# tp7/Sushi

Measured on NVIDIA H100. Metric: subtitle_events_per_s, higher is better.
Workload: dtype f32

## Files before the change

### sushi_b200/csrc/sb_fused2.cu

```cuda
#include "sb_internal.h"
#include <cmath>
#include <cstdlib>
#include <vector>

#include "sb_fused_common.cuh"
#include "sb_fft_smem.cuh"

using namespace sb;
using namespace sbf;

#ifndef SB_V2_SPECIAL_PREFETCH
#define SB_V2_SPECIAL_PREFETCH 1
#endif

namespace {

constexpr int QB = 16384;
constexpr int QT = 512;
constexpr int QNW = QT / 32;
constexpr int Q4 = QB / 4;
constexpr int QBLK = 256;
constexpr int QROW = kQuadRowF2 / 2;
__host__ __device__ constexpr int qa(int i) { return i < Q4 ? (i >> 8) * (2 * QBLK) + (i & (QBLK - 1)) : 2 * Q4; }
__host__ __device__ constexpr int qm(int i) { return i < Q4 ? qa(i) + QBLK : 2 * Q4 + 1; }
// ... 379 lines not shown
        int rq = 0, rs = 0;
        double dq = 0.0, ds = 0.0;
#pragma unroll
        for (int i = 0; i < 8; ++i) {
            const float wq = f_w0q + (is_u8 ? (float)rq : (float)dq);
            const float sit = fmaf(cc[i], f_scale, fmaf(f_b, is_u8 ? (float)rs : (float)ds, f_k0));
            const float num = fmaxf((wq + f_tsq) - 2.0f * sit, 0.0f);
            const float pr = wq * f_tsq;
            const float v = fminf(num * rsqrt_fast(pr), 1.0f);
            if (interior) { vf[c][i] = v; tmin = fminf(tmin, v); }
            else if (j0 + i >= jlo && j0 + i < jhi) { vf[c][i] = v; tmin = fminf(tmin, v); }
            else vf[c][i] = kSent;
            if (is_u8) {
                const int lo = (int)((lo8 >> (8 * i)) & 0xffu), hi = (int)((hi8 >> (8 * i)) & 0xffu);
                rq += hi * hi - lo * lo; rs += hi - lo;
            } else if (j0 + i + n < img_n) {
                const double lo = (double)img32[j0 + i], hi = (double)img32[j0 + i + n];
                dq += hi * hi - lo * lo; ds += hi - lo;
            }
        }
    }
    const float my_min = tmin;
#pragma unroll
    for (int o = 16; o > 0; o >>= 1) tmin = fminf(tmin, __shfl_xor_sync(0xffffffffu, tmin, o));
    if (lane == 0) s_min[warp] = tmin;
    if (is_u8) fence_proxy_async();
    csync<ID>();
    after_read();
    float bmin = s_min[0];
#pragma unroll
    for (int w = 1; w < NW; ++w) bmin = fminf(bmin, s_min[w]);
    const float thr = curve_out ? 1.5f : bmin + kScreenMargin;

    unsigned long long cand = 0;
    if (my_min <= thr) {
#pragma unroll
        for (int c = 0; c < ROUNDS; ++c)
#pragma unroll
            for (int i = 0; i < 8; ++i) cand |= (vf[c][i] <= thr) ? (1ull << (c * 8 + i)) : 0ull;
    }
    unsigned long long best = ~0ull;
    while (cand) {
        const int bit = __ffsll((long long)cand) - 1;
        cand &= cand - 1;
        const int m = (bit >> 3) * LAGS_PER_ROUND + tid * 8 + (bit & 7);
        const int64_t j = j_blk + m;
        const int jj = m >> 2;
        const int ca = (jj & 15) * kDA + ((jj >> 4) & 15) * kDB + 2 * (jj >> 8);
        const C2 E = buf.ld(ca), O = buf.ld(ca + 1);
        const float2 w = make_float2(kC32[jj >> 8], kS32[jj >> 8]);
        const bool second = (m & 2) != 0;
        const float er = second ? E.r.y : E.r.x, ei = second ? E.i.y : E.i.x, orr = second ? O.r.y : O.r.x, oi = second ? O.i.y : O.i.x;
        const float xr = fmaf(orr, w.x, fmaf(oi, -w.y, er)), xi = fmaf(orr, w.y, fmaf(oi, w.x, ei));
        const double cc = (double)((m & 1) ? xi : xr) * scale;
        const double2 p_hi = ipfx[j + n], p_lo = ipfx[j];
        const float v = sqdiff_exact(cc, p_hi.x - p_lo.x, p_hi.y - p_lo.y, a, b, tsum, tsq, n_ab);
        if (curve_out) curve_out[d.curveOff + (j - jlo)] = v;
        const unsigned long long key = ((unsigned long long)__float_as_uint(v) << 32) | (unsigned int)(j - jlo);
        best = key < best ? key : best;
    }
#pragma unroll
    for (int o = 16; o > 0; o >>= 1) {
        const unsigned long long other = __shfl_xor_sync(0xffffffffu, best, o);
        best = other < best ? other : best;
    }
    if (lane == 0) s_best[warp] = best;
    csync<ID>();
    if (tid == 0) {
        for (int w = 1; w < NW; ++w) best = s_best[w] < best ? s_best[w] : best;
        if (best != ~0ull) atomicMin(keys + it.q, best);
    }
}

template <int ID, typename AfterRead>
__device__ __forceinline__ void finish_item_v3(const Item& it, int tid, const Smem& sm, unsigned long long* s_bar, unsigned bar_parity,
                                               float* s_min, int2* s_w0, int64_t img_n,
                                               unsigned long long* __restrict__ keys, float* __restrict__ curve_out,
                                               AfterRead after_read, RunSink sink) {
    constexpr int NW = QNW, LB = QB, RUNS = 4;
    constexpr float kSent = 3.0e38f;
    const Buf& buf = sm.buf;
    const int lane = tid & 31, warp = tid >> 5;
    const QueryDesc& d = it.d;
    const int64_t j_blk = it.j_blk, n = d.tlen, jlo = d.lag0, jhi = d.lag0 + d.nlags;
    const double2* s_qc = reinterpret_cast<const double2*>(sm.end + kQueryConstOff());
    const double tsum = s_qc[0].x, tsq = s_qc[0].y, a = s_qc[1].x, b = s_qc[1].y;
    const double n_ab = (double)n * a * b;
    const double scale = 1.0 / (double)(2 * QB);
    const double k_const = a * tsum - n_ab;
    const float f_tsq = (float)tsq, f_b = (float)b;
    const float m2s = -2.0f * (float)scale, m2b = -2.0f * f_b;
    const bool interior = j_blk >= jlo && j_blk + LB <= jhi;
    const int64_t jt = j_blk + 32 * tid;
    constexpr float kRunQ = 7.0f * 255.0f * 255.0f;
    const float f_bm = fmaxf(f_b, 255.0f - f_b);
    const float f_delta = 1.02f * 7.0f * f_bm * f_bm + 1024.0f;
    const float rt = sqrtf(f_tsq), m_rt = kScreenMargin * rt, sat = (1.0f - kScreenMargin) * rt;
    const int ech = 8 * (tid & 1) * kDA + ((tid >> 1) & 15) * kDB + 2 * warp;
    const float wc = kC32[warp], ws = kS32[warp];

    mbar_wait(s_bar, bar_parity);
    unsigned lw[8], hw[8];
    {
        const uint4 l0 = *reinterpret_cast<const uint4*>(sm.lo + 32 * tid), l1 = *reinterpret_cast<const uint4*>(sm.lo + 32 * tid + 16);
        lw[0] = l0.x; lw[1] = l0.y; lw[2] = l0.z; lw[3] = l0.w; lw[4] = l1.x; lw[5] = l1.y; lw[6] = l1.z; lw[7] = l1.w;
        const int hi_off = (int)((j_blk + n) & 15);
        const uint4 h0 = *reinterpret_cast<const uint4*>(sm.hi + 32 * tid), h1 = *reinterpret_cast<const uint4*>(sm.hi + 32 * tid + 16),
                    h2 = *reinterpret_cast<const uint4*>(sm.hi + 32 * tid + 32);
        unsigned w[12] = {h0.x, h0.y, h0.z, h0.w, h1.x, h1.y, h1.z, h1.w, h2.x, h2.y, h2.z, h2.w};
        unsigned v[10], u[9];
#pragma unroll
        for (int k = 0; k < 10; ++k) v[k] = (hi_off & 8) ? w[k + 2] : w[k];
#pragma unroll
        for (int k = 0; k < 9; ++k) u[k] = (hi_off & 4) ? v[k + 1] : v[k];
        const unsigned sh = (unsigned)(hi_off & 3) * 8u;
#pragma unroll
        for (int k = 0; k < 8; ++k) hw[k] = __funnelshift_r(u[k], u[k + 1], sh);
    }
    int tq[RUNS], ts[RUNS];
#pragma unroll
    for (int r = 0; r < RUNS; ++r) {
        tq[r] = (int)__dp4a(hw[2 * r], hw[2 * r], __dp4a(hw[2 * r + 1], hw[2 * r + 1], 0u)) - (int)__dp4a(lw[2 * r], lw[2 * r], __dp4a(lw[2 * r + 1], lw[2 * r + 1], 0u));
        ts[r] = (int)__dp4a(hw[2 * r], 0x01010101u, __dp4a(hw[2 * r + 1], 0x01010101u, 0u)) - (int)__dp4a(lw[2 * r], 0x01010101u, __dp4a(lw[2 * r + 1], 0x01010101u, 0u));
    }
    const int Tq = (tq[0] + tq[1]) + (tq[2] + tq[3]), Ts = (ts[0] + ts[1]) + (ts[2] + ts[3]);
    int iq = Tq, is = Ts;
#pragma unroll
    for (int o = 1; o < 32; o <<= 1) {
        const int uq = __shfl_up_sync(0xffffffffu, iq, o), us = __shfl_up_sync(0xffffffffu, is, o);
        if (lane >= o) { iq += uq; is += us; }
    }
    const double2 b_lo = sm.base[warp * 2], b_hi = sm.base[warp * 2 + 1];
    const double Wq = b_hi.y - b_lo.y, Ws = b_hi.x - b_lo.x;
    const double Cw = Wq + tsq - 2.0 * (b * Ws + k_const);
    const int bi2 = 2 * (int)b;
    float run_lb[RUNS];
    float tmin = kSent;
    int oq = iq - Tq, os = is - Ts;
#pragma unroll
    for (int r = 0; r < RUNS; ++r) {
        s_w0[r * QT + tid] = make_int2(os, oq);
        const float f_w0q = (float)(Wq + 0.25 + (double)oq);
        const float f_A = (float)(Cw + (double)(oq - bi2 * os));
        float cc[8];
#pragma unroll
        for (int e = 0; e < 2; ++e) {
            const C2 E = buf.ld(ech + kDA * (2 * r + e)), O = buf.ld(ech + kDA * (2 * r + e) + 1);
            const float2 xr = fma2(O.r, bc(wc), fma2(O.i, bc(-ws), E.r));
            const float2 xi = fma2(O.r, bc(ws), fma2(O.i, bc(wc), E.i));
            cc[4 * e + 0] = xr.x; cc[4 * e + 1] = xi.x; cc[4 * e + 2] = xr.y; cc[4 * e + 3] = xi.y;
        }
        const float cmax = fmaxf(fmaxf(fmaxf(cc[0], cc[1]), fmaxf(cc[2], cc[3])), fmaxf(fmaxf(cc[4], cc[5]), fmaxf(cc[6], cc[7])));
        const int64_t j0 = jt + 8 * r;
        const bool some = interior || (j0 < jhi && j0 + 8 > jlo);
        const bool inside = interior || (j0 >= jlo && j0 + 8 <= jhi);
        const float lbn = fmaf(cmax, m2s, f_A - f_delta), ubn = lbn + 2.0f * f_delta;
        const float lbv = lbn * rsqrt_fast(f_w0q + kRunQ) * 0.999999f;
        run_lb[r] = !some ? kSent : (lbn >= 0.f ? lbv : -kSent);
        const float ubv = ubn * rsqrt_fast(f_w0q - kRunQ) * 1.000001f;
        if (inside && f_w0q > 4.0f * kRunQ && ubn >= 0.f) tmin = fminf(tmin, ubv);
        oq += tq[r]; os += ts[r];
    }
#pragma unroll
    for (int o = 16; o > 0; o >>= 1) tmin = fminf(tmin, __shfl_xor_sync(0xffffffffu, tmin, o));
    if (lane == 0) s_min[warp] = tmin;
    fence_proxy_async();
    csync<ID>();
    static_assert(NW == 16, "block minimum over 16 warps");
    float bmin = s_min[lane & (NW - 1)];
#pragma unroll
    for (int o = NW / 2; o > 0; o >>= 1) bmin = fminf(bmin, __shfl_xor_sync(0xffffffffu, bmin, o));
    const float thr = bmin + m_rt;
    const bool all = curve_out != nullptr || !(bmin < sat);
    unsigned left = 0;
#pragma unroll
    for (int r = 0; r < RUNS; ++r) left |= (run_lb[r] <= thr || (all && run_lb[r] < kSent)) ? (1u << r) : 0u;
    if (left && sink.recs != nullptr && !all) {
#pragma unroll 1
        for (int r = 0; r < RUNS; ++r) {
            if (!((left >> r) & 1u)) continue;
            const int slot = atomicAdd(sink.s_cnt, 1);
            if (slot >= kRunSlots) break;
            float cc[8];
            const int k3 = warp;
#pragma unroll
            for (int e = 0; e < 2; ++e) {
                const C2 E = buf.ld(ech + kDA * (2 * r + e)), O = buf.ld(ech + kDA * (2 * r + e) + 1);
                const float2 w = make_float2(kC32[k3], kS32[k3]);
                const float2 xr = fma2(O.r, bc(w.x), fma2(O.i, bc(-w.y), E.r));
                const float2 xi = fma2(O.r, bc(w.y), fma2(O.i, bc(w.x), E.i));
                cc[4 * e + 0] = xr.x; cc[4 * e + 1] = xi.x; cc[4 * e + 2] = xr.y; cc[4 * e + 3] = xi.y;
            }
            float4* r4 = reinterpret_cast<float4*>(sink.recs + slot);
            const int64_t j0 = jt + 8 * r;
            *reinterpret_cast<int4*>(r4) = make_int4(it.q, 1, (int)(unsigned)(j0 & 0xffffffffll), (int)(j0 >> 32));
            r4[1] = make_float4(cc[0], cc[1], cc[2], cc[3]);
            r4[2] = make_float4(cc[4], cc[5], cc[6], cc[7]);
            left &= ~(1u << r);
        }
    }
    unsigned long long best = ~0ull;
    if (__any_sync(0xffffffffu, left != 0u)) {
        unsigned cand = 0;
#pragma unroll 1
        for (int r = 0; r < RUNS; ++r) {
            const bool sel = (left >> r) & 1u;
            if (!__any_sync(0xffffffffu, sel)) continue;
            const int64_t j0 = jt + 8 * r;
            float cc[8];
#pragma unroll
            for (int e = 0; e < 2; ++e) {
                const C2 E = buf.ld(ech + kDA * (2 * r + e)), O = buf.ld(ech + kDA * (2 * r + e) + 1);
                const float2 xr = fma2(O.r, bc(wc), fma2(O.i, bc(-ws), E.r));
                const float2 xi = fma2(O.r, bc(ws), fma2(O.i, bc(wc), E.i));
                cc[4 * e + 0] = xr.x; cc[4 * e + 1] = xi.x; cc[4 * e + 2] = xr.y; cc[4 * e + 3] = xi.y;
            }
            const unsigned long long lo8 = *reinterpret_cast<const unsigned long long*>(sm.lo + 32 * tid + 8 * r);
            const int hb = (int)((j_blk + n) & 15) + 32 * tid + 8 * r;
            const unsigned long long h0 = *reinterpret_cast<const unsigned long long*>(sm.hi + (hb & ~7));
            const unsigned long long h1 = *reinterpret_cast<const unsigned long long*>(sm.hi + (hb & ~7) + 8);
            const unsigned shb = (unsigned)(hb & 7) * 8u;
            const unsigned long long hi8 = shb ? ((h0 >> shb) | (h1 << (64u - shb))) : h0;
            const int2 off = s_w0[r * QT + tid];
            const float f_w0q = (float)(Wq + 0.25 + (double)off.y);
            const float f_A = (float)(Cw + (double)(off.y - bi2 * off.x));
            float v8[8];
            float vmin = kSent;
            int rq = 0, rs = 0;
#pragma unroll
            for (int i = 0; i < 8; ++i) {
                const float frq = (float)rq;
                const float num = fmaf(cc[i], m2s, fmaf(m2b, (float)rs, f_A + frq));
                const float v = num * rsqrt_fast(f_w0q + frq);
                const bool valid = sel && j0 + i >= jlo && j0 + i < jhi;
                v8[i] = valid ? v : kSent;
                vmin = fminf(vmin, v8[i]);
                const int lo = (int)((lo8 >> (8 * i)) & 0xffu), hi = (int)((hi8 >> (8 * i)) & 0xffu);
                const int dd = hi - lo;
                rq += (hi + lo) * dd; rs += dd;
            }
#pragma unroll
            for (int o = 16; o > 0; o >>= 1) vmin = fminf(vmin, __shfl_xor_sync(0xffffffffu, vmin, o));
            const float thrw = fminf(thr, vmin + m_rt);
#pragma unroll
            for (int i = 0; i < 8; ++i) cand |= (v8[i] < kSent && (v8[i] <= thrw || all)) ? (1u << (r * 8 + i)) : 0u;
        }
        while (cand) {
            const int bit = __ffs((int)cand) - 1;
            cand &= cand - 1;
            const int r = bit >> 3, i = bit & 7;
            const int m = 32 * tid + bit;
            const int64_t j = j_blk + m;
            const int jj = m >> 2;
            const int ca = (jj & 15) * kDA + ((jj >> 4) & 15) * kDB + 2 * (jj >> 8);
            const C2 E = buf.ld(ca), O = buf.ld(ca + 1);
            const float2 w = make_float2(kC32[jj >> 8], kS32[jj >> 8]);
            const bool second = (m & 2) != 0;
            const float er = second ? E.r.y : E.r.x, ei = second ? E.i.y : E.i.x, orr = second ? O.r.y : O.r.x, oi = second ? O.i.y : O.i.x;
            const float xr = fmaf(orr, w.x, fmaf(oi, -w.y, er)), xi = fmaf(orr, w.y, fmaf(oi, w.x, ei));
            const double cc = (double)((m & 1) ? xi : xr) * scale;
            const unsigned long long lo8 = *reinterpret_cast<const unsigned long long*>(sm.lo + 32 * tid + 8 * r);
            const int hb = (int)((j_blk + n) & 15) + 32 * tid + 8 * r;
            const unsigned long long h0 = *reinterpret_cast<const unsigned long long*>(sm.hi + (hb & ~7));
            const unsigned long long h1 = *reinterpret_cast<const unsigned long long*>(sm.hi + (hb & ~7) + 8);
            const unsigned shb = (unsigned)(hb & 7) * 8u;
            const unsigned long long hi8 = shb ? ((h0 >> shb) | (h1 << (64u - shb))) : h0;
            const unsigned long long keep = i ? (~0ull >> (8 * (8 - i))) : 0ull;
            const unsigned la = (unsigned)(lo8 & keep), lb = (unsigned)((lo8 & keep) >> 32), ha = (unsigned)(hi8 & keep), hb2 = (unsigned)((hi8 & keep) >> 32);
            const int rq = (int)__dp4a(ha, ha, __dp4a(hb2, hb2, 0u)) - (int)__dp4a(la, la, __dp4a(lb, lb, 0u));
            const int rs = (int)__dp4a(ha, 0x01010101u, __dp4a(hb2, 0x01010101u, 0u)) - (int)__dp4a(la, 0x01010101u, __dp4a(lb, 0x01010101u, 0u));
            const int2 off = s_w0[r * QT + tid];
            const double wsum = (Ws + (double)off.x) + (double)rs, wsq = (Wq + (double)off.y) + (double)rq;
            const float v = sqdiff_exact(cc, wsum, wsq, a, b, tsum, tsq, n_ab);
            if (curve_out) curve_out[d.curveOff + (j - jlo)] = v;
            const unsigned long long key = ((unsigned long long)__float_as_uint(v) << 32) | (unsigned int)(j - jlo);
            best = key < best ? key : best;
        }
        if (best != ~0ull) atomicMin(keys + it.q, best);
    }
    fence_proxy_async();
    csync<ID>();
    after_read();
}

template <typename S> struct QueryStreams { const float4* Xhat; int64_t nblk; const S* img; int64_t img_n; const double2* ipfx; const double2* tpfx; };
template <typename S>
__device__ __forceinline__ QueryStreams<S> select_streams(const StreamEntry* streams, const int2* slots, int q) {
    const int2 sl = slots[q];
    const StreamEntry si = streams[sl.x];
    return {reinterpret_cast<const float4*>(si.specq), si.nblk, static_cast<const S*>(si.raw), si.n, si.pfx, streams[sl.y].pfx};
}
#define SB_SELECT_STREAMS(q) do { const QueryStreams<S> qs__ = select_streams<S>(streams, slots, (q)); \
    Xhat = qs__.Xhat; nblk = qs__.nblk; img = qs__.img; img_n = qs__.img_n; ipfx = qs__.ipfx; tpfx = qs__.tpfx; } while (0)

template <typename S, int EPI, bool MULTI = false>
__global__ void __launch_bounds__(QT, 1)
k_match_packed(const float4* __restrict__ That, int64_t part_first,
               const float4* __restrict__ Xhat, int64_t nblk,
               const S* __restrict__ img, int64_t img_n,
               const double2* __restrict__ ipfx, const double2* __restrict__ tpfx,
               const QueryDesc* __restrict__ desc, const int* __restrict__ item_query, int64_t item_first,
               PackedTables tab, unsigned long long* __restrict__ keys, float* __restrict__ curve_out,
               RunRecord* __restrict__ recs, int* __restrict__ rec_count,
               const StreamEntry* __restrict__ streams = nullptr, const int2* __restrict__ slots = nullptr) {
    constexpr int T = QT, NW = QNW;
    constexpr bool is_u8 = sizeof(S) == 1;
    extern __shared__ __align__(16) unsigned char smem_raw[];
    const Smem sm(smem_raw);
    unsigned long long* s_bar = reinterpret_cast<unsigned long long*>(sm.end);
    unsigned long long* s_best = s_bar + 1;
    float* s_min = reinterpret_cast<float*>(s_best + NW);
    int* s_cnt = reinterpret_cast<int*>(sm.end + kRunCountOff());
    const RunSink sink = {EPI == 3 && recs ? recs + (size_t)blockIdx.x * kRunSlots : nullptr, s_cnt};
    float4* s_sp = reinterpret_cast<float4*>(sm.end + kSmallBytes);
    int2* s_w0 = EPI >= 2 && is_u8 ? reinterpret_cast<int2*>(sm.end + kSmallBytes + kSpecialBytes) : nullptr;
    const Buf& buf = sm.buf;

    const int tid = threadIdx.x, lane = tid & 31, warp = tid >> 5;
    const Item it(desc, item_query, item_first, blockIdx.x);
    const QueryDesc& d = it.d;
    if constexpr (MULTI) SB_SELECT_STREAMS(it.q);

    if (is_u8) {
        if (tid == 0) mbar_init(s_bar, 1);
        stage_inputs<EPI == 3>(it, tid, reinterpret_cast<const uint8_t*>(img), img_n, ipfx, sm, s_bar);
    }
    if (EPI == 3 && tid == 96) *s_cnt = 0;
    if (EPI >= 2 && tid == 64) query_constants<S>(reinterpret_cast<double2*>(sm.end + kQueryConstOff()), d, img_n, ipfx, tpfx);

    {
        int P = d.P;
        if (it.k + P > nblk) P = (int)(nblk - it.k);
        typedef Rows R;
        const float4* tp = That + (d.partBase - part_first) * (int64_t)R::STRIDE;
        const float4* xp = Xhat + it.k * (int64_t)R::STRIDE;
        const float2 wbase = __ldg(tab.wb + tid);
        const int tm = (T - tid) & (T - 1);
        const int col = phys(tid), mcol = phys(tm);
        const bool sp_pref = EPI >= 2 && SB_V2_SPECIAL_PREFETCH && special_fits(d.P, 1);
        if (sp_pref && warp == NW - 1) special_prefetch(s_sp, tp, xp, d.P, 1, it.k, nblk, lane);
        constexpr int U = 4;
#pragma unroll 1
        for (int half = 0; half < 2; ++half) {
            const int i0 = R::unit(tid, half * U);
            QuadAcc acc[U];
#pragma unroll
            for (int u = 0; u < U; ++u) acc[u].zero();
#pragma unroll 1
            for (int p = 0; p < P; ++p) {
                const float4* t = tp + (int64_t)p * R::STRIDE;
                const float4* x = xp + (int64_t)p * R::STRIDE;
                float4 ta[U], tmm[U], xa[U], xm[U];
#pragma unroll
                for (int u = 0; u < U; ++u) {
                    R::load(t, i0 + u * R::USTEP, ta[u], tmm[u]);
                    R::load(x, i0 + u * R::USTEP, xa[u], xm[u]);
                }
#pragma unroll
                for (int u = 0; u < U; ++u) acc[u].mac(ta[u], tmm[u], xa[u], xm[u]);
            }
#pragma unroll
            for (int u = 0; u < U; ++u) {
                const int uu = half * U + u;
                const float c = wbase.x * kC64[uu] - wbase.y * kS64[uu];
                const float s = wbase.x * kS64[uu] + wbase.y * kC64[uu];
                C2 lo, hi;
                pack_quad(acc[u].aR, acc[u].aI, acc[u].mR, acc[u].mI, c, s, lo, hi);
                buf.st(col + kUU * uu, lo);
                if (tid != 0) buf.st(mcol + kUU * (15 - uu), hi);
                else if (uu != 0) buf.st(mcol + kUU * (16 - uu), hi);
            }
        }
        if (warp == NW - 1) {
            if (sp_pref) {
                cp_async_commit_wait_all();
                __syncwarp();
                const C2 lo = special_from_smem(s_sp, d.P, 0, lane);
                if (lane == 0) buf.st(phys(Q4), lo);
            } else {
                const C2 lo = special_quad(tp, xp, P, lane);
                if (lane == 0) buf.st(phys(Q4), lo);
            }
        }
    }
    csync<0>();

    fft_passes_dif<0>(buf, tid, tab, is_u8);
    if constexpr (EPI == 3) finish_item_v3<0>(it, tid, sm, s_bar, 0u, s_min, s_w0, img_n, keys, curve_out, [] {}, sink);
    else finish_item<S, 0>(it, tid, sm, s_bar, 0u, s_best, s_min, img, img_n, ipfx, tpfx, keys, curve_out, [] {});
    if (EPI == 3 && rec_count && tid == 0) rec_count[blockIdx.x] = *s_cnt < kRunSlots ? *s_cnt : kRunSlots;
}

constexpr int kParkF4 = 16 * QT;

__device__ __forceinline__ void unpark(const float4* pk, const Buf& buf, int col, int mcol, int tid) {
#pragma unroll
    for (int uu = 0; uu < 8; ++uu) {
        const C2 lo = from4(park_ld(pk + (2 * uu) * QT)), hi = from4(park_ld(pk + (2 * uu + 1) * QT));
        buf.st(col + kUU * uu, lo);
        if (tid != 0) buf.st(mcol + kUU * (15 - uu), hi);
        else if (uu != 0) buf.st(mcol + kUU * (16 - uu), hi);
    }
}

template <typename S, int EPI, bool MULTI = false>
__global__ void __launch_bounds__(QT, 1)
k_match_pair(const float4* __restrict__ That, int64_t part_first,
             const float4* __restrict__ Xhat, int64_t nblk,
             const S* __restrict__ img, int64_t img_n,
             const double2* __restrict__ ipfx, const double2* __restrict__ tpfx,
             const QueryDesc* __restrict__ desc, const int* __restrict__ pair_query, int64_t pair_first, int64_t n_pairs,
             float4* __restrict__ park, int* __restrict__ park_busy, int park_slots,
             PackedTables tab, unsigned long long* __restrict__ keys, float* __restrict__ curve_out,
             RunRecord* __restrict__ recs, int* __restrict__ rec_count,
             const StreamEntry* __restrict__ streams = nullptr, const int2* __restrict__ slots = nullptr) {
    constexpr int T = QT, NW = QNW;
    constexpr bool is_u8 = sizeof(S) == 1;
    extern __shared__ __align__(16) unsigned char smem_raw[];
    const Smem sm(smem_raw);
    unsigned long long* s_bar = reinterpret_cast<unsigned long long*>(sm.end);
    unsigned long long* s_best = s_bar + 1;
    float* s_min = reinterpret_cast<float*>(s_best + NW);
    int* s_slot = reinterpret_cast<int*>(s_min + NW);
    int* s_cnt = reinterpret_cast<int*>(sm.end + kRunCountOff());
    int* s_next_q = reinterpret_cast<int*>(sm.end + kNextOff());
    QueryDesc* s_next_d = reinterpret_cast<QueryDesc*>(sm.end + kNextOff() + 16);
    float4* s_sp = reinterpret_cast<float4*>(sm.end + kSmallBytes);
    int2* s_w0 = EPI >= 2 && is_u8 ? reinterpret_cast<int2*>(sm.end + kSmallBytes + kSpecialBytes) : nullptr;
    const Buf& buf = sm.buf;

    const int tid = threadIdx.x, lane = tid & 31, warp = tid >> 5;
    if (tid == 64) *s_slot = park_acquire(park_busy, park_slots, (int)(blockIdx.x % (unsigned)park_slots));
    if (is_u8 && tid == 0) mbar_init(s_bar, 1);
    if (EPI == 3 && tid == 32) *s_cnt = 0;
    csync<0>();
    float4* const pk = park + (size_t)*s_slot * kParkF4 + tid;
    const int tm = (T - tid) & (T - 1);
    const int col = phys(tid), mcol = phys(tm);
    const float2 wbase = __ldg(tab.wb + tid);
    unsigned phase = 0;

    constexpr bool kPersistent = EPI == 3, kPrefetch = kPersistent;
    int64_t pi = blockIdx.x;
    do {
    const bool first = !kPrefetch || pi == (int64_t)blockIdx.x;
    const int q = first ? __ldg(pair_query + pi) : *s_next_q;
    const QueryDesc d = first ? desc[q] : *s_next_d;
    if constexpr (MULTI) SB_SELECT_STREAMS(q);
    const int64_t pi_next = pi + gridDim.x;
    int q_next = 0;
    if (kPrefetch && tid == 32 && pi_next < n_pairs) q_next = __ldg(pair_query + pi_next);
    const int lp = (int)(pair_first + pi - d.groupBase);
    const bool has2 = 2 * lp + 1 < d.nk;
    const Item it0(d, q, d.k0 + 2 * lp), it1(d, q, d.k0 + 2 * lp + 1);
    const RunSink sink = {EPI == 3 && recs ? recs + (size_t)pi * kRunSlots : nullptr, s_cnt};

    if (is_u8) stage_inputs<EPI == 3>(it0, tid, reinterpret_cast<const uint8_t*>(img), img_n, ipfx, sm, s_bar);
    if (EPI >= 2 && tid == 64) query_constants<S>(reinterpret_cast<double2*>(sm.end + kQueryConstOff()), d, img_n, ipfx, tpfx);
    C2 sp1 = {make_float2(0.f, 0.f), make_float2(0.f, 0.f)};
    {
        typedef Rows R;
        const int64_t k = it0.k;
        const float4* tp = That + (d.partBase - part_first) * (int64_t)R::STRIDE;
        const float4* xp = Xhat + k * (int64_t)R::STRIDE;
        const bool sp_pref = EPI >= 2 && SB_V2_SPECIAL_PREFETCH && special_fits(d.P, 2);
        if (sp_pref && warp == NW - 1) special_prefetch(s_sp, tp, xp, d.P, 2, k, nblk, lane);
        constexpr int U = 2;
#pragma unroll 1
        for (int grp = 0; grp < 8 / U; ++grp) {
            const int i0 = R::unit(tid, grp * U);
            QuadAcc a0[U], a1[U];
            float4 xa[U], xm[U];
#pragma unroll
            for (int u = 0; u < U; ++u) {
                a0[u].zero(); a1[u].zero();
                R::load(xp, i0 + u * R::USTEP, xa[u], xm[u]);
            }
#pragma unroll 2
            for (int p = 0; p < d.P; ++p) {
                const float4* t = tp + (int64_t)p * R::STRIDE;
                const float4* x = xp + (int64_t)(p + 1) * R::STRIDE;
                const bool next_row = k + p + 1 < nblk;
                float4 ta[U], tmm[U], xna[U], xnm[U];
#pragma unroll
                for (int u = 0; u < U; ++u) {
                    R::load(t, i0 + u * R::USTEP, ta[u], tmm[u]);
                    R::loadp(x, i0 + u * R::USTEP, next_row, xna[u], xnm[u]);
                }
#pragma unroll
                for (int u = 0; u < U; ++u) {
                    a0[u].mac(ta[u], tmm[u], xa[u], xm[u]);
                    a1[u].mac(ta[u], tmm[u], xna[u], xnm[u]);
                    xa[u] = xna[u]; xm[u] = xnm[u];
                }
            }
#pragma unroll
            for (int u = 0; u < U; ++u) {
                const int uu = grp * U + u;
                const float c = wbase.x * kC64[uu] - wbase.y * kS64[uu];
                const float s = wbase.x * kS64[uu] + wbase.y * kC64[uu];
                C2 lo, hi;
                pack_quad(a0[u].aR, a0[u].aI, a0[u].mR, a0[u].mI, c, s, lo, hi);
                buf.st(col + kUU * uu, lo);
                if (tid != 0) buf.st(mcol + kUU * (15 - uu), hi);
                else if (uu != 0) buf.st(mcol + kUU * (16 - uu), hi);
                pack_quad(a1[u].aR, a1[u].aI, a1[u].mR, a1[u].mI, c, s, lo, hi);
                park_st(pk + (2 * uu) * QT, make_float4(lo.r.x, lo.r.y, lo.i.x, lo.i.y));
                park_st(pk + (2 * uu + 1) * QT, make_float4(hi.r.x, hi.r.y, hi.i.x, hi.i.y));
            }
        }
        if (warp == NW - 1) {
            if (sp_pref) {
                cp_async_commit_wait_all();
                __syncwarp();
                const C2 lo = special_from_smem(s_sp, d.P, 0, lane);
                if (lane == 0) buf.st(phys(Q4), lo);
                if (has2) sp1 = special_from_smem(s_sp, d.P, 1, lane);
            } else {
                int P0 = d.P; if (k + P0 > nblk) P0 = (int)(nblk - k);
                const C2 lo = special_quad(tp, xp, P0, lane);
                if (lane == 0) buf.st(phys(Q4), lo);
                if (has2) {
                    int P1 = d.P; if (k + 1 + P1 > nblk) P1 = (int)(nblk - k - 1);
                    sp1 = special_quad(tp, xp + R::STRIDE, P1, lane);
                }
            }
        }
    }
    csync<0>();
    if (kPrefetch && tid == 32 && pi_next < n_pairs) {
        *s_next_q = q_next;
        const float4* src = reinterpret_cast<const float4*>(desc + q_next);
        static_assert(sizeof(QueryDesc) == 80, "five 16-byte copies");
#pragma unroll
        for (int k = 0; k < 5; ++k) cp_async16(reinterpret_cast<float4*>(s_next_d) + k, src + k);
    }

    fft_passes_dif<0>(buf, tid, tab, true);
    auto stage_second = [&] { if (is_u8 && has2) stage_inputs<EPI == 3>(it1, tid, reinterpret_cast<const uint8_t*>(img), img_n, ipfx, sm, s_bar); };
    if constexpr (EPI == 3) finish_item_v3<0>(it0, tid, sm, s_bar, phase & 1u, s_min, s_w0, img_n, keys, curve_out, stage_second, sink);
    else finish_item<S, 0>(it0, tid, sm, s_bar, phase & 1u, s_best, s_min, img, img_n, ipfx, tpfx, keys, curve_out, stage_second);
    ++phase;

    if (has2) {
        unpark(pk, buf, col, mcol, tid);
        if (tid == (NW - 1) * 32) buf.st(phys(Q4), sp1);
        csync<0>();
        fft_passes_dif<0>(buf, tid, tab, is_u8);
        if constexpr (EPI == 3) finish_item_v3<0>(it1, tid, sm, s_bar, phase & 1u, s_min, s_w0, img_n, keys, curve_out, [] {}, sink);
        else finish_item<S, 0>(it1, tid, sm, s_bar, phase & 1u, s_best, s_min, img, img_n, ipfx, tpfx, keys, curve_out, [] {});
        ++phase;
    }
    if (EPI == 3 && rec_count && tid == 32) { rec_count[pi] = *s_cnt < kRunSlots ? *s_cnt : kRunSlots; *s_cnt = 0; }
    } while (kPersistent && (pi += gridDim.x) < n_pairs);
    csync<0>();
    if (tid == 64) park_release(park_busy + *s_slot);
}

template <typename S, bool MULTI = false>
__global__ void __launch_bounds__(128)
k_finish_runs(const RunRecord* __restrict__ recs, const int* __restrict__ rec_count, int64_t n_ctas,
              const QueryDesc* __restrict__ desc, const double2* __restrict__ ipfx, int64_t img_n,
              const double2* __restrict__ tpfx, unsigned long long* __restrict__ keys,
              const StreamEntry* __restrict__ streams = nullptr, const int2* __restrict__ slots = nullptr) {
    const int64_t idx = (int64_t)blockIdx.x * blockDim.x + threadIdx.x;
    const int64_t cta = idx / kRunSlots;
    const int slot = (int)(idx - cta * kRunSlots);
    if (cta >= n_ctas || slot >= rec_count[cta]) return;
    const float4* r4 = reinterpret_cast<const float4*>(recs + cta * kRunSlots + slot);
    const int4 head = *reinterpret_cast<const int4*>(r4);
    const float4 c0 = r4[1], c1 = r4[2];
    const float cc[8] = {c0.x, c0.y, c0.z, c0.w, c1.x, c1.y, c1.z, c1.w};
    const int q = head.x;
    const int64_t j0 = (int64_t)(unsigned)head.z | ((int64_t)head.w << 32);
    if constexpr (MULTI) {
        const int2 sl = slots[q];
        ipfx = streams[sl.x].pfx; img_n = streams[sl.x].n; tpfx = streams[sl.y].pfx;
    }
    const QueryDesc d = desc[q];
    const int64_t n = d.tlen, jlo = d.lag0, jhi = d.lag0 + d.nlags;
    const double2 t_hi = tpfx[d.toff + n], t_lo = tpfx[d.toff];
    const double tsum = t_hi.x - t_lo.x, tsq = t_hi.y - t_lo.y;
    const double a = (double)Acc<S>::centre(ipfx[img_n].x, (double)img_n);
    const double b = (double)Acc<S>::centre(tsum, (double)n);
    const double n_ab = (double)n * a * b;
    const double scale = 1.0 / (double)(2 * QB);
    unsigned long long best = ~0ull;
#pragma unroll 1
    for (int i = 0; i < 8; ++i) {
        const int64_t j = j0 + i;
        if (j < jlo || j >= jhi) continue;
        const double2 p_hi = ipfx[j + n], p_lo = ipfx[j];
        const float v = sqdiff_exact((double)cc[i] * scale, p_hi.x - p_lo.x, p_hi.y - p_lo.y, a, b, tsum, tsq, n_ab);
        const unsigned long long key = ((unsigned long long)__float_as_uint(v) << 32) | (unsigned int)(j - jlo);
        best = key < best ? key : best;
    }
    if (best != ~0ull) atomicMin(keys + q, best);
}

__global__ void k_fill_pair_query(const QueryDesc* __restrict__ desc, int q_begin, int64_t pair_first, int* __restrict__ pair_query, int group) {
    const int q = q_begin + blockIdx.x;
    const int64_t base = desc[q].groupBase - pair_first;
    const int np = (desc[q].nk + group - 1) / group;
    for (int i = threadIdx.x; i < np; i += blockDim.x) pair_query[base + i] = q;
}

template <typename S, int MODE, bool MULTI = false>
__global__ void __launch_bounds__(Cfg<14>::T, 1)
k_forward_quad(const S* __restrict__ src, int64_t src_n, const double2* __restrict__ pfx,
               const QueryDesc* __restrict__ desc, int q_begin, int q_end, int64_t row_first,
               FusedTables tab, float4* __restrict__ out,
               const StreamEntry* __restrict__ streams = nullptr, const int2* __restrict__ slots = nullptr,
               const int2* __restrict__ row_list = nullptr, int64_t rows = -1) {
    typedef Cfg<14> C;
    constexpr int N = C::N, T = C::T, B = C::N;
    constexpr int NT2 = C::R2 * 32, NT3 = C::R3 * 32;
    extern __shared__ __align__(16) unsigned char smem_raw[];
    float2* buf = reinterpret_cast<float2*>(smem_raw);
    float2* s_t2 = buf + pad(N) + 1;
    float2* s_a3 = s_t2 + NT2;
    float2* s_b3 = s_a3 + NT3;
    int* s_q = reinterpret_cast<int*>(s_b3 + NT3);
    const int tid = threadIdx.x;
    for (int i = tid; i < NT2; i += T) s_t2[i] = __ldg(tab.t2 + i);
    for (int i = tid; i < NT3; i += T) { s_a3[i] = __ldg(tab.a3 + i); s_b3[i] = __ldg(tab.b3 + i); }

    for (int64_t item = blockIdx.x; rows < 0 ? item == blockIdx.x : item < rows; item += gridDim.x) {
        const S* xs = src;
        const double2* xpfx = pfx;
        float4* xout = out;
        int64_t off, len;
        float centre;
        int64_t row = row_first + item, out_row = item;
        if constexpr (MULTI && MODE == 0) {
            const int2 rl = row_list[item];
            const StreamEntry se = streams[rl.x];
            xs = static_cast<const S*>(se.raw); xpfx = se.pfx;
            xout = reinterpret_cast<float4*>(se.specq);
            row = out_row = rl.y;
            off = row * B;
            len = se.n - off; if (len > 2 * B) len = 2 * B; if (len < 0) len = 0;
            centre = Acc<S>::centre(xpfx[se.n].x, (double)se.n);
        } else if (MODE == 0) {
            off = row * B;
            len = src_n - off; if (len > 2 * B) len = 2 * B; if (len < 0) len = 0;
            centre = Acc<S>::centre(pfx[src_n].x, (double)src_n);
        } else {
            int lo = q_begin, n = q_end - q_begin;
            while (n > 1) {
                const int s = (n + T - 1) / T, m = (n + s - 1) / s;
                auto le = [&](int t) { return t == 0 || (t < m && desc[lo + t * s].partBase <= row); };
                if (le(tid) && !le(tid + 1)) *s_q = tid;
                __syncthreads();
                const int c = *s_q;
                __syncthreads();
                lo += c * s;
                n = c == m - 1 ? n - c * s : s;
            }
            const int q = lo;
            const QueryDesc d = desc[q];
            if constexpr (MULTI) { xs = static_cast<const S*>(streams[slots[q].y].raw); xpfx = streams[slots[q].y].pfx; }
            const int64_t seg0 = (row - d.partBase) * B;
            off = d.toff + seg0;
            len = d.tlen - seg0; if (len > B) len = B;
            centre = Acc<S>::centre(xpfx[d.toff + d.tlen].x - xpfx[d.toff].x, (double)d.tlen);
        }
        const S* x = xs + off;
#pragma unroll
        for (int k = 0; k < B / T; ++k) {
            const int n = tid + k * T;
            const int64_t i0 = 2 * (int64_t)n;
            const float a = i0 < len ? (float)x[i0] - centre : 0.f;
            const float b = i0 + 1 < len ? (float)x[i0 + 1] - centre : 0.f;
            buf[pad(n)] = make_float2(a, -b);
        }
        __syncthreads();
        ifft_smem<C::R3, false>(buf, s_t2, s_a3, s_b3);
        auto bins = [&](int k, float2& xk, float2& xbk) {
            const float2 zk = buf[pad(k)];
            const float2 zp = buf[pad(k == 0 ? 0 : B - k)];
            const float2 A = make_float2(zk.x, -zk.y), P = make_float2(zp.x, zp.y);
            const float2 xe = make_float2(0.5f * (A.x + P.x), 0.5f * (A.y + P.y));
            const float2 dd = make_float2(A.x - P.x, A.y - P.y);
            const float2 xo = make_float2(0.5f * dd.y, -0.5f * dd.x);
            const float2 w = __ldg(tab.w + k);
            const float2 tv = cmul(make_float2(w.x, -w.y), xo);
            xk = make_float2(xe.x + tv.x, xe.y + tv.y);
            xbk = make_float2(xe.x - tv.x, -(xe.y - tv.y));
        };
        float4* o = xout + out_row * QROW;
        for (int i = tid; i <= Q4; i += T) {
            float2 x_i, x_bi, x_h, x_hb;
            bins(i, x_i, x_bi);
            bins(B / 2 - i, x_h, x_hb);
            o[qa(i)] = make_float4(x_i.x, x_hb.x, x_i.y, x_hb.y);
            o[qm(i)] = make_float4(x_bi.x, x_h.x, x_bi.y, x_h.y);
        }
        __syncthreads();
    }
}

size_t forward_smem_bytes14() {
    typedef Cfg<14> C;
    return ((size_t)(C::N + (C::N >> 5) + 1) + C::R2 * 32 + 2 * C::R3 * 32) * sizeof(float2) + 64;
}

static_assert(8 + QNW * 8 + QNW * 4 + 4 <= kRunCountOff() && kRunCountOff() + 4 <= kNextOff() &&
              kNextOff() + 16 + (int)sizeof(QueryDesc) <= kQueryConstOff() && kQueryConstOff() + 32 <= kSmallBytes, "small shared-memory area");
size_t packed_smem_bytes(int epi = 1) {
    return epi >= 2 ? kSmemCommon + kSmallBytes + kSpecialBytes + (size_t)kRounds * QT * sizeof(int2)
                    : kSmemCommon + kSmallBytes;
}

constexpr int kPackedTableCount = 3;
std::vector<float> packed_table_values(size_t (&off)[kPackedTableCount]) {
    const double pi = 3.14159265358979323846;
    const size_t nb = 512 * 2, nd1 = 8 * 512 * 4, nd2 = 8 * 32 * 4;
    off[0] = 0; off[1] = nb; off[2] = nb + nd1;
    std::vector<float> h(off[2] + nd2);
    auto pairs = [&](size_t at, int K, double N) {
        for (int a = 0; a < 8; ++a)
            for (int k = 0; k < K; ++k)
                for (int e = 0; e < 2; ++e) {
                    const double ang = 2.0 * pi * (double)((2 * a + e) * k) / N;
                    h[at + ((size_t)a * K + k) * 4 + 2 * e] = (float)cos(ang); h[at + ((size_t)a * K + k) * 4 + 2 * e + 1] = (float)sin(ang);
                }
    };
    for (int t = 0; t < 512; ++t) { h[off[0] + 2 * t] = (float)cos(pi * t / QB); h[off[0] + 2 * t + 1] = (float)sin(pi * t / QB); }
    pairs(off[1], 512, 8192.0);
    pairs(off[2], 32, 512.0);
    return h;
}

PackedTables packed_tables_at(const float* base, const size_t (&off)[kPackedTableCount]) {
    PackedTables t;
    t.wb = reinterpret_cast<const float2*>(base + off[0]);
    t.d1 = reinterpret_cast<const float4*>(base + off[1]);
    t.d2 = reinterpret_cast<const float4*>(base + off[2]);
    return t;
}

#ifndef SB_EMULATE
float* g_ptab_dev = nullptr;
PackedTables g_ptab;

int ensure_packed_tables(PackedTables* out) {
    if (!g_ptab_dev) {
        size_t off[kPackedTableCount];
        const std::vector<float> h = packed_table_values(off);
        SB_CUDA(cudaMalloc(&g_ptab_dev, h.size() * sizeof(float)));
        SB_CUDA(cudaMemcpy(g_ptab_dev, h.data(), h.size() * sizeof(float), cudaMemcpyHostToDevice));
        g_ptab = packed_tables_at(g_ptab_dev, off);
    }
    *out = g_ptab;
    return SB_OK;
}

__global__ void k_fill_item_query2(const QueryDesc* __restrict__ desc, int q_begin, int64_t item_first,
                                   int* __restrict__ item_query) {
    const int q = q_begin + blockIdx.x;
    const int64_t base = desc[q].itemBase - item_first;
    const int nk = desc[q].nk;
    for (int i = threadIdx.x; i < nk; i += blockDim.x) item_query[base + i] = q;
}

int* g_item_query2 = nullptr;
int64_t g_item_query2_cap = 0;

template <typename S, int MODE, bool MULTI = false>
int launch_forward_quad_typed(const sb_stream* src, const QueryDesc* d_desc, int q_begin, int q_end,
                              int64_t row_first, int64_t rows, float2* out, const MultiArgs* m = nullptr,
                              const int2* row_list = nullptr) {
    Ctx& c = ctx();
    FusedTables tab;
    SB_TRY(fused_tables(&tab));
    static bool attr_set = false;
    const size_t smem = forward_smem_bytes14();
    if (!attr_set) {
        SB_CUDA(cudaFuncSetAttribute(k_forward_quad<S, MODE, MULTI>, cudaFuncAttributeMaxDynamicSharedMemorySize, (int)smem));
        attr_set = true;
    }
    const int64_t grid = std::min<int64_t>(rows, c.sm_count);
    k_forward_quad<S, MODE, MULTI><<<(unsigned)grid, Cfg<14>::T, smem, c.stream>>>(
        static_cast<const S*>(src->d_raw), src->n, src->d_pfx, d_desc, q_begin, q_end, row_first, tab,
        reinterpret_cast<float4*>(out), MULTI ? m->d_streams : nullptr, MULTI ? m->d_slots : nullptr, row_list, rows);
    SB_CUDA(cudaGetLastError());
    return SB_OK;
}

int ensure_item_query(int64_t n) {
    if (g_item_query2_cap < n) {
        cudaStreamSynchronize(ctx().stream);
        cudaFree(g_item_query2); g_item_query2 = nullptr; g_item_query2_cap = 0;
        SB_CUDA(cudaMalloc(&g_item_query2, sizeof(int) * (size_t)n));
        g_item_query2_cap = n;
    }
    return SB_OK;
}

RunRecord* g_run_recs = nullptr;
int* g_run_count = nullptr;
int64_t g_run_cap = 0;
constexpr int64_t kRunChunk = 1 << 19;

int ensure_run_records(int64_t n_ctas) {
    if (g_run_cap < n_ctas) {
        cudaStreamSynchronize(ctx().stream);
        cudaFree(g_run_recs); cudaFree(g_run_count); g_run_recs = nullptr; g_run_count = nullptr; g_run_cap = 0;
        SB_CUDA(cudaMalloc(&g_run_recs, sizeof(RunRecord) * (size_t)n_ctas * kRunSlots));
        SB_CUDA(cudaMalloc(&g_run_count, sizeof(int) * (size_t)n_ctas));
        g_run_cap = n_ctas;
    }
    return SB_OK;
}

float4* g_park = nullptr;
int* g_park_busy = nullptr;
int g_park_slots = 0;

int ensure_park() {
    Ctx& c = ctx();
    if (g_park_slots != c.sm_count) {
        cudaStreamSynchronize(c.stream);
        cudaFree(g_park); cudaFree(g_park_busy); g_park = nullptr; g_park_busy = nullptr; g_park_slots = 0;
        SB_CUDA(cudaMalloc(&g_park, sizeof(float4) * kParkF4 * (size_t)c.sm_count));
        SB_CUDA(cudaMalloc(&g_park_busy, sizeof(int) * (size_t)c.sm_count));
        SB_CUDA(cudaMemsetAsync(g_park_busy, 0, sizeof(int) * (size_t)c.sm_count, c.stream));
        g_park_slots = c.sm_count;
    }
    return SB_OK;
}

const sb_stream kNoStream{};

template <typename S, bool MULTI>
int launch_finish_runs(const sb_stream* image, const sb_stream* tmpl, const QueryDesc* d_desc, int64_t n_ctas, unsigned long long* d_keys,
                       const MultiArgs* m) {
    Ctx& c = ctx();
    const int64_t threads = n_ctas * kRunSlots;
    k_finish_runs<S, MULTI><<<(unsigned)((threads + 127) / 128), 128, 0, c.stream>>>(g_run_recs, g_run_count, n_ctas, d_desc, image->d_pfx, image->n,
                                                                                   tmpl->d_pfx, d_keys, MULTI ? m->d_streams : nullptr,
                                                                                   MULTI ? m->d_slots : nullptr);
    c.launches += 1;
    SB_CUDA(cudaGetLastError());
    return SB_OK;
}

template <typename S, int EPI, bool MULTI>
int launch_packed_typed(const sb_stream* image, const sb_stream* tmpl, const float2* d_parts, int64_t part_first,
                        const QueryDesc* d_desc, int64_t item_first, int64_t n_items, const PackedTables& tab,
                        unsigned long long* d_keys, float* d_curve, const MultiArgs* m) {
    Ctx& c = ctx();
    static bool attr_set = false;
    const size_t smem = packed_smem_bytes(EPI);
    if (!attr_set) {
        SB_CUDA(cudaFuncSetAttribute(k_match_packed<S, EPI, MULTI>, cudaFuncAttributeMaxDynamicSharedMemorySize, (int)smem));
        attr_set = true;
    }
    const bool records = EPI == 3 && d_curve == nullptr;
    const int64_t max_grid = records ? kRunChunk : (int64_t)1 << 30;
    for (int64_t i0 = 0; i0 < n_items; i0 += max_grid) {
        const int64_t ni = std::min<int64_t>(max_grid, n_items - i0);
        if (records) SB_TRY(ensure_run_records(ni));
        k_match_packed<S, EPI, MULTI><<<(unsigned)ni, QT, smem, c.stream>>>(
            reinterpret_cast<const float4*>(d_parts), part_first, reinterpret_cast<const float4*>(image->d_specq), image->nblkq,
            static_cast<const S*>(image->d_raw), image->n, image->d_pfx, tmpl->d_pfx, d_desc, g_item_query2 + i0, item_first + i0,
            tab, d_keys, d_curve, records ? g_run_recs : nullptr, records ? g_run_count : nullptr,
            MULTI ? m->d_streams : nullptr, MULTI ? m->d_slots : nullptr);
        if (records) SB_TRY((launch_finish_runs<S, MULTI>(image, tmpl, d_desc, ni, d_keys, m)));
    }
    SB_CUDA(cudaGetLastError());
    return SB_OK;
}

template <typename S, int EPI, bool MULTI>
int launch_pair_typed(const sb_stream* image, const sb_stream* tmpl, const float2* d_parts, int64_t part_first,
                      const QueryDesc* d_desc, int64_t pair_first, int64_t n_pairs, const PackedTables& tab,
                      unsigned long long* d_keys, float* d_curve, const MultiArgs* m) {
    Ctx& c = ctx();
    static bool attr_set = false;
    const size_t smem = packed_smem_bytes(EPI) + 16;
    if (!attr_set) {
        SB_CUDA(cudaFuncSetAttribute(k_match_pair<S, EPI, MULTI>, cudaFuncAttributeMaxDynamicSharedMemorySize, (int)smem));
        attr_set = true;
    }
    const bool records = EPI == 3 && d_curve == nullptr;
    const int64_t max_grid = records ? kRunChunk : (int64_t)1 << 30;
    for (int64_t i0 = 0; i0 < n_pairs; i0 += max_grid) {
        const int64_t ni = std::min<int64_t>(max_grid, n_pairs - i0);
        if (records) SB_TRY(ensure_run_records(ni));
        const int64_t grid = EPI == 3 ? std::min<int64_t>(ni, c.sm_count) : ni;
        k_match_pair<S, EPI, MULTI><<<(unsigned)grid, QT, smem, c.stream>>>(
            reinterpret_cast<const float4*>(d_parts), part_first, reinterpret_cast<const float4*>(image->d_specq), image->nblkq,
            static_cast<const S*>(image->d_raw), image->n, image->d_pfx, tmpl->d_pfx, d_desc, g_item_query2 + i0, pair_first + i0, ni,
            g_park, g_park_busy, g_park_slots, tab, d_keys, d_curve, records ? g_run_recs : nullptr, records ? g_run_count : nullptr,
            MULTI ? m->d_streams : nullptr, MULTI ? m->d_slots : nullptr);
        SB_CUDA(cudaGetLastError());
        if (records) SB_TRY((launch_finish_runs<S, MULTI>(image, tmpl, d_desc, ni, d_keys, m)));
    }
    return SB_OK;
}

#define SB_DISPATCH_MATCH1(FN, M, dtype, ...) \
    ((dtype) != SB_U8        ? FN<float, 1, M>(__VA_ARGS__) \
     : ctx().epilogue == 3   ? FN<uint8_t, 3, M>(__VA_ARGS__) : FN<uint8_t, 1, M>(__VA_ARGS__))
#define SB_DISPATCH_MATCH(FN, image, tmpl, multi, ...) \
    ((multi) ? SB_DISPATCH_MATCH1(FN, true, (multi)->dtype, &kNoStream, &kNoStream, __VA_ARGS__, multi) \
             : SB_DISPATCH_MATCH1(FN, false, (image)->dtype, image, tmpl, __VA_ARGS__, multi))

}

namespace sb {

int launch_match_packed(const sb_stream* image, const sb_stream* tmpl, const float2* d_parts, int64_t part_first,
                        const QueryDesc* d_desc, int q_begin, int q_end, int64_t item_first, int64_t n_items,
                        unsigned long long* d_keys, float* d_curve, const MultiArgs* multi) {
    Ctx& c = ctx();
    PackedTables tab;
    SB_TRY(ensure_packed_tables(&tab));
    SB_TRY(ensure_item_query(n_items));
    k_fill_item_query2<<<(unsigned)(q_end - q_begin), 128, 0, c.stream>>>(d_desc, q_begin, item_first, g_item_query2);
    c.launches += 1;
    return SB_DISPATCH_MATCH(launch_packed_typed, image, tmpl, multi, d_parts, part_first, d_desc, item_first, n_items, tab, d_keys, d_curve);
}

int launch_match_pair(const sb_stream* image, const sb_stream* tmpl, const float2* d_parts, int64_t part_first,
                      const QueryDesc* d_desc, int q_begin, int q_end, int64_t pair_first, int64_t n_pairs,
                      unsigned long long* d_keys, float* d_curve, const MultiArgs* multi) {
    Ctx& c = ctx();
    PackedTables tab;
    SB_TRY(ensure_packed_tables(&tab));
    SB_TRY(ensure_item_query(n_pairs));
    SB_TRY(ensure_park());
    k_fill_pair_query<<<(unsigned)(q_end - q_begin), 128, 0, c.stream>>>(d_desc, q_begin, pair_first, g_item_query2, 2);
    c.launches += 1;
    return SB_DISPATCH_MATCH(launch_pair_typed, image, tmpl, multi, d_parts, part_first, d_desc, pair_first, n_pairs, tab, d_keys, d_curve);
}

int launch_block_spectra_quad(const sb_stream* s, int64_t k_first, int64_t rows, float2* out) {
    return s->dtype == SB_U8 ? launch_forward_quad_typed<uint8_t, 0>(s, nullptr, 0, 0, k_first, rows, out)
                             : launch_forward_quad_typed<float, 0>(s, nullptr, 0, 0, k_first, rows, out);
}

int launch_block_spectra_quad_multi(const MultiArgs& m, const int2* d_row_list, int64_t n_rows) {
    return m.dtype == SB_U8 ? launch_forward_quad_typed<uint8_t, 0, true>(&kNoStream, nullptr, 0, 0, 0, n_rows, nullptr, &m, d_row_list)
                            : launch_forward_quad_typed<float, 0, true>(&kNoStream, nullptr, 0, 0, 0, n_rows, nullptr, &m, d_row_list);
}

int launch_part_spectra_quad(const sb_stream* tmpl, const QueryDesc* d_desc, int q_begin, int q_end,
                             int64_t part_first, int64_t rows, float2* out, const MultiArgs* multi) {
    if (multi)
        return multi->dtype == SB_U8 ? launch_forward_quad_typed<uint8_t, 1, true>(&kNoStream, d_desc, q_begin, q_end, part_first, rows, out, multi)
                                     : launch_forward_quad_typed<float, 1, true>(&kNoStream, d_desc, q_begin, q_end, part_first, rows, out, multi);
    return tmpl->dtype == SB_U8 ? launch_forward_quad_typed<uint8_t, 1>(tmpl, d_desc, q_begin, q_end, part_first, rows, out)
                                : launch_forward_quad_typed<float, 1>(tmpl, d_desc, q_begin, q_end, part_first, rows, out);
}

void packed_release_tables() {
    if (g_ptab_dev) cudaFree(g_ptab_dev);
    g_ptab_dev = nullptr;
    cudaFree(g_item_query2); g_item_query2 = nullptr; g_item_query2_cap = 0;
    cudaFree(g_run_recs); cudaFree(g_run_count); g_run_recs = nullptr; g_run_count = nullptr; g_run_cap = 0;
    cudaFree(g_park); cudaFree(g_park_busy); g_park = nullptr; g_park_busy = nullptr; g_park_slots = 0;
}

}
#else
}
#endif
```

Measured before the change: 48810.

## Make EPI3 packed match kernel persistent with atomic work queue and descriptor prefetch

For the EPI==3 path, the packed match kernel now launches one block per SM and loops, pulling further items from a global atomic counter. The next item's query descriptor is prefetched into shared memory with cp.async while the FFT passes run. The mbarrier phase is carried across iterations and run counts are reset for each item. The aim is to remove per-block launch and setup cost and overlap descriptor fetches, at the price of a serial atomic fetch per item and less ability to hide tail imbalance. It relies on new shared-memory offsets (kNextOff) and an Item constructor that are not shown.

```diff
diff --git a/sushi_b200/csrc/sb_fused2.cu b/sushi_b200/csrc/sb_fused2.cu
--- a/sushi_b200/csrc/sb_fused2.cu
+++ b/sushi_b200/csrc/sb_fused2.cu
@@ -705,7 +705,8 @@
                const QueryDesc* __restrict__ desc, const int* __restrict__ item_query, int64_t item_first,
                PackedTables tab, unsigned long long* __restrict__ keys, float* __restrict__ curve_out,
                RunRecord* __restrict__ recs, int* __restrict__ rec_count,
-               const StreamEntry* __restrict__ streams = nullptr, const int2* __restrict__ slots = nullptr) {
+               const StreamEntry* __restrict__ streams = nullptr, const int2* __restrict__ slots = nullptr,
+               int64_t n_items = -1, int* __restrict__ item_next = nullptr) {
     constexpr int T = QT, NW = QNW;
     constexpr bool is_u8 = sizeof(S) == 1;
     extern __shared__ __align__(16) unsigned char smem_raw[];
@@ -714,21 +715,35 @@
     unsigned long long* s_best = s_bar + 1;
     float* s_min = reinterpret_cast<float*>(s_best + NW);
     int* s_cnt = reinterpret_cast<int*>(sm.end + kRunCountOff());
-    const RunSink sink = {EPI == 3 && recs ? recs + (size_t)blockIdx.x * kRunSlots : nullptr, s_cnt};
+    int* s_next_q = reinterpret_cast<int*>(sm.end + kNextOff());
+    int64_t* s_next_i = reinterpret_cast<int64_t*>(sm.end + kNextOff() + 8);
+    QueryDesc* s_next_d = reinterpret_cast<QueryDesc*>(sm.end + kNextOff() + 16);
     float4* s_sp = reinterpret_cast<float4*>(sm.end + kSmallBytes);
     int2* s_w0 = EPI >= 2 && is_u8 ? reinterpret_cast<int2*>(sm.end + kSmallBytes + kSpecialBytes) : nullptr;
     const Buf& buf = sm.buf;
 
     const int tid = threadIdx.x, lane = tid & 31, warp = tid >> 5;
-    const Item it(desc, item_query, item_first, blockIdx.x);
+    const bool persistent = EPI == 3 && n_items >= 0;
+    if (is_u8 && tid == 0) mbar_init(s_bar, 1);
+    if (EPI == 3 && tid == 0) *s_cnt = 0;
+    unsigned phase = 0;
+    int64_t local = blockIdx.x;
+    bool first = true;
+    do {
+    const int q = first ? __ldg(item_query + local) : *s_next_q;
+    const QueryDesc dq = first ? desc[q] : *s_next_d;
+    const Item it(dq, q, dq.k0 + (item_first + local - dq.itemBase));
     const QueryDesc& d = it.d;
     if constexpr (MULTI) SB_SELECT_STREAMS(it.q);
-
-    if (is_u8) {
-        if (tid == 0) mbar_init(s_bar, 1);
-        stage_inputs<EPI == 3>(it, tid, reinterpret_cast<const uint8_t*>(img), img_n, ipfx, sm, s_bar);
-    }
-    if (EPI == 3 && tid == 96) *s_cnt = 0;
+    int64_t next = n_items;
+    int q_next = 0;
+    if (persistent && tid == 32) {
+        next = (int64_t)gridDim.x + atomicAdd(item_next, 1);
+        if (next < n_items) q_next = __ldg(item_query + next);
+    }
+    const RunSink sink = {EPI == 3 && recs ? recs + (size_t)local * kRunSlots : nullptr, s_cnt};
+
+    if (is_u8) stage_inputs<EPI == 3>(it, tid, reinterpret_cast<const uint8_t*>(img), img_n, ipfx, sm, s_bar);
     if (EPI >= 2 && tid == 64) query_constants<S>(reinterpret_cast<double2*>(sm.end + kQueryConstOff()), d, img_n, ipfx, tpfx);
 
     {
@@ -787,11 +802,24 @@
         }
     }
     csync<0>();
+    if (persistent && tid == 32) *s_next_i = next;
+    if (persistent && tid == 32 && next < n_items) {
+        *s_next_q = q_next;
+        const float4* src = reinterpret_cast<const float4*>(desc + q_next);
+#pragma unroll
+        for (int k = 0; k < 5; ++k) cp_async16(reinterpret_cast<float4*>(s_next_d) + k, src + k);
+    }
 
     fft_passes_dif<0>(buf, tid, tab, is_u8);
-    if constexpr (EPI == 3) finish_item_v3<0>(it, tid, sm, s_bar, 0u, s_min, s_w0, img_n, keys, curve_out, [] {}, sink);
-    else finish_item<S, 0>(it, tid, sm, s_bar, 0u, s_best, s_min, img, img_n, ipfx, tpfx, keys, curve_out, [] {});
-    if (EPI == 3 && rec_count && tid == 0) rec_count[blockIdx.x] = *s_cnt < kRunSlots ? *s_cnt : kRunSlots;
+    if constexpr (EPI == 3) finish_item_v3<0>(it, tid, sm, s_bar, phase & 1u, s_min, s_w0, img_n, keys, curve_out, [] {}, sink);
+    else finish_item<S, 0>(it, tid, sm, s_bar, phase & 1u, s_best, s_min, img, img_n, ipfx, tpfx, keys, curve_out, [] {});
+    ++phase;
+    if (EPI == 3 && tid == 0) {
+        if (rec_count) rec_count[local] = *s_cnt < kRunSlots ? *s_cnt : kRunSlots;
+        *s_cnt = 0;
+    }
+    first = false;
+    } while (persistent && (local = *s_next_i) < n_items);
 }
 
 constexpr int kParkF4 = 16 * QT;
@@ -1169,6 +1197,7 @@
 
 int* g_item_query2 = nullptr;
 int64_t g_item_query2_cap = 0;
+int* g_item_next = nullptr;
 
 template <typename S, int MODE, bool MULTI = false>
 int launch_forward_quad_typed(const sb_stream* src, const QueryDesc* d_desc, int q_begin, int q_end,
@@ -1198,6 +1227,7 @@
         SB_CUDA(cudaMalloc(&g_item_query2, sizeof(int) * (size_t)n));
         g_item_query2_cap = n;
     }
+    if (!g_item_next) SB_CUDA(cudaMalloc(&g_item_next, sizeof(int)));
     return SB_OK;
 }
 
@@ -1265,11 +1295,13 @@
     for (int64_t i0 = 0; i0 < n_items; i0 += max_grid) {
         const int64_t ni = std::min<int64_t>(max_grid, n_items - i0);
         if (records) SB_TRY(ensure_run_records(ni));
-        k_match_packed<S, EPI, MULTI><<<(unsigned)ni, QT, smem, c.stream>>>(
+        const int64_t grid = EPI == 3 ? std::min<int64_t>(ni, c.sm_count) : ni;
+        if (EPI == 3) SB_CUDA(cudaMemsetAsync(g_item_next, 0, sizeof(int), c.stream));
+        k_match_packed<S, EPI, MULTI><<<(unsigned)grid, QT, smem, c.stream>>>(
             reinterpret_cast<const float4*>(d_parts), part_first, reinterpret_cast<const float4*>(image->d_specq), image->nblkq,
             static_cast<const S*>(image->d_raw), image->n, image->d_pfx, tmpl->d_pfx, d_desc, g_item_query2 + i0, item_first + i0,
             tab, d_keys, d_curve, records ? g_run_recs : nullptr, records ? g_run_count : nullptr,
-            MULTI ? m->d_streams : nullptr, MULTI ? m->d_slots : nullptr);
+            MULTI ? m->d_streams : nullptr, MULTI ? m->d_slots : nullptr, EPI == 3 ? ni : (int64_t)-1, g_item_next);
         if (records) SB_TRY((launch_finish_runs<S, MULTI>(image, tmpl, d_desc, ni, d_keys, m)));
     }
     SB_CUDA(cudaGetLastError());
@@ -1363,6 +1395,7 @@
     if (g_ptab_dev) cudaFree(g_ptab_dev);
     g_ptab_dev = nullptr;
     cudaFree(g_item_query2); g_item_query2 = nullptr; g_item_query2_cap = 0;
+    cudaFree(g_item_next); g_item_next = nullptr;
     cudaFree(g_run_recs); cudaFree(g_run_count); g_run_recs = nullptr; g_run_count = nullptr; g_run_cap = 0;
     cudaFree(g_park); cudaFree(g_park_busy); g_park = nullptr; g_park_busy = nullptr; g_park_slots = 0;
 }
```

New measurement: 48470 (median of 6 runs). About the same (-0.7%).
